# Spandan7724/Audio-Watermarking-Deep-Learning-Watermarks-for-Authenticating-Speech

Measured on AMD Instinct MI355X. Metric: 1-s@16kHz clips/sec (gen+det+loss fwd-bwd), higher is better.
Workload: dtype f32; 1 GPU; main16 train step: Generator+Detector+6 losses fwd-bwd + Adam, B=256 clips/GPU x 1 GPU, 1-s @ 16 kHz, message_bits=16 (BASELINE configs[2]); batch_per_gpu=256, global_batch=256, clip_len=16000, optimizer=fused flat Adam (wm_adam_step), parallelism=single

## Files before the change

### audio-watermarking-deep-learning-watermarks-for-authenticating-speech_amd/csrc/fft_lds.hpp

```cpp
#pragma once
#include "wm_common.hpp"

namespace wm {

__device__ __forceinline__ float2 cmul(float2 a, float2 b) { return make_float2(a.x * b.x - a.y * b.y, a.x * b.y + a.y * b.x); }

template <int LOGN>
__device__ __forceinline__ void fft_dif(float2* z, const float2* tw, int tid) {
    constexpr int N = 1 << LOGN;
#pragma unroll 1
    for (int st = 0; st < LOGN; ++st) {
        const int lm = LOGN - 1 - st, m = 1 << lm;
        for (int j = tid; j < N / 2; j += 256) {
            const int pos = j & (m - 1), i0 = ((j >> lm) << (lm + 1)) + pos, i1 = i0 + m;
            const float2 a = z[i0], b = z[i1], w = tw[pos << st];
            z[i0] = make_float2(a.x + b.x, a.y + b.y);
            z[i1] = cmul(make_float2(a.x - b.x, a.y - b.y), w);
        }
        __syncthreads();
    }
}
__device__ __forceinline__ double2 cmul(double2 a, double2 b) { return make_double2(a.x * b.x - a.y * b.y, a.x * b.y + a.y * b.x); }
template <int LOGN>
__device__ __forceinline__ void fft_dif(double2* z, const double2* tw, int tid) {
    constexpr int N = 1 << LOGN;
#pragma unroll 1
    for (int st = 0; st < LOGN; ++st) {
        const int lm = LOGN - 1 - st, m = 1 << lm;
        for (int j = tid; j < N / 2; j += 256) {
            const int pos = j & (m - 1), i0 = ((j >> lm) << (lm + 1)) + pos, i1 = i0 + m;
            const double2 a = z[i0], b = z[i1], w = tw[pos << st];
            z[i0] = make_double2(a.x + b.x, a.y + b.y);
            z[i1] = cmul(make_double2(a.x - b.x, a.y - b.y), w);
        }
        __syncthreads();
    }
}
template <int LOGN>
__device__ __forceinline__ int brev(int k) { return (int)(__brev((unsigned)k) >> (32 - LOGN)); }

}
```

### audio-watermarking-deep-learning-watermarks-for-authenticating-speech_amd/csrc/postproc.hip

```cpp
#include "wm_common.hpp"
using namespace wm;

namespace {

constexpr int kMaxTaps = 128;

__global__ __launch_bounds__(256) void postproc_fwd_kernel(const float* __restrict__ d_in, const float* __restrict__ taps,
                                                           int ntaps, float thr, float max_rms, float eps, int stages,
                                                           float* __restrict__ f_out, float* __restrict__ d_out,
                                                           float* __restrict__ stats, int T) {
    extern __shared__ __align__(16) float smem[];
    float* xs = smem;
    float* ks = smem + T + kMaxTaps;
    __shared__ float scratch[8];
    const int b = blockIdx.x, tid = threadIdx.x, pad = (ntaps - 1) / 2;
    const float* x = d_in + (size_t)b * T;
    const bool do_fir = stages & 1;
    for (int i = tid; i < T + 2 * pad; i += 256) {
        const int t = i - pad;
        xs[i] = (t >= 0 && t < T) ? x[t] : 0.f;
    }
    if (tid < ntaps) ks[tid] = taps[tid];
    __syncthreads();
    float ss = 0.f;
    for (int t = tid; t < T; t += 256) {
        float f;
        if (do_fir) {
            f = 0.f;
            for (int j = 0; j < ntaps; ++j) f = fmaf(ks[j], xs[t + j], f);
        } else {
            f = xs[t + pad];
        }
        if (f_out) f_out[(size_t)b * T + t] = f;
        const float cl = (stages & 2) ? fminf(fmaxf(f, -thr), thr) : f;
        d_out[(size_t)b * T + t] = cl;
        ss = fmaf(cl, cl, ss);
    }
    if (stages & 4) {
        const float tot = block_sum<4>(ss, scratch);
        const float cur = sqrtf(tot / (float)T + eps);
        const float gain = fminf(max_rms / cur, 1.0f);
        if (tid == 0 && stats) { stats[2 * b] = cur; stats[2 * b + 1] = gain; }
        for (int t = tid; t < T; t += 256) d_out[(size_t)b * T + t] *= gain;
    } else if (tid == 0 && stats) {
        stats[2 * b] = 0.f; stats[2 * b + 1] = 1.f;
    }
}

__global__ __launch_bounds__(256) void postproc_bwd_kernel(const float* __restrict__ g, const float* __restrict__ f_in,
                                                           const float* __restrict__ stats, const float* __restrict__ taps,
                                                           int ntaps, float thr, float max_rms, int stages,
                                                           float* __restrict__ d_raw, int T) {
    extern __shared__ __align__(16) float smem[];
    float* gs = smem;
    float* ks = smem + T + kMaxTaps;
    __shared__ float scratch[8];
    const int b = blockIdx.x, tid = threadIdx.x, pad = (ntaps - 1) / 2;
    const float* gb = g + (size_t)b * T;
    const float* fb = f_in + (size_t)b * T;
    if (tid < ntaps) ks[tid] = taps[tid];
    for (int i = tid; i < pad; i += 256) { gs[i] = 0.f; gs[pad + T + i] = 0.f; }
    float cur = 0.f, gain = 1.f;
    if (stages & 4) { cur = stats[2 * b]; gain = stats[2 * b + 1]; }
    float dot = 0.f;
    if ((stages & 4) && gain < 1.0f) {
        float acc = 0.f;
        for (int t = tid; t < T; t += 256) {
            const float f = fb[t];
            const float cl = (stages & 2) ? fminf(fmaxf(f, -thr), thr) : f;
            acc = fmaf(gb[t], cl, acc);
        }
        dot = block_sum<4>(acc, scratch);
    }
    const float r = max_rms / cur;
    const float kk = dot / ((float)T * cur * cur);
    for (int t = tid; t < T; t += 256) {
        const float f = fb[t];
        const float cl = (stages & 2) ? fminf(fmaxf(f, -thr), thr) : f;
        float dd = gb[t];
        if ((stages & 4) && gain < 1.0f) dd = r * (dd - cl * kk);
        if ((stages & 2) && !(f >= -thr && f <= thr)) dd = 0.f;
        gs[pad + t] = dd;
    }
    __syncthreads();
    for (int t = tid; t < T; t += 256) {
        float acc;
        if (stages & 1) {
            acc = 0.f;
            for (int j = 0; j < ntaps; ++j) acc = fmaf(ks[j], gs[t + 2 * pad - j], acc);
        } else {
            acc = gs[pad + t];
        }
        d_raw[(size_t)b * T + t] = acc;
    }
}

__global__ void embed_gather_kernel(const float* __restrict__ table, const long long* __restrict__ message,
                                    float* __restrict__ vec, int B, int nrows, int* __restrict__ err) {
    const int i = blockIdx.x * blockDim.x + threadIdx.x;
    if (i >= B * 64) return;
    const long long m = message[i >> 6];
    if (m < 0 || m >= nrows) { if (err) *err = 1; vec[i] = 0.f; return; }
    vec[i] = table[(size_t)m * 64 + (i & 63)];
}

__global__ __launch_bounds__(256) void embed_scatter_add_kernel(float* __restrict__ dtable, const long long* __restrict__ message,
                                                                const float* __restrict__ dvec, int B, int nrows) {
    const int lane = threadIdx.x & 63, b = blockIdx.x * 4 + (threadIdx.x >> 6);
    if (b >= B) return;
    const long long m = message[b];
    if (m < 0 || m >= nrows) return;
    float* row = dtable + (size_t)m * 64 + lane;
    float acc = 0.f;
    bool owner = false;
    for (int k0 = 0; k0 < B; k0 += 64) {
        const int idx = k0 + lane;
        const long long id = idx < B ? message[idx] : -1;
        unsigned long long hit = __ballot(id == m);
        if (k0 + 64 <= b) {
            if (hit) return;
            continue;
        }
        if (!owner) {
            const int sh = b - k0;
            if (hit & ((1ull << sh) - 1ull)) return;
            hit &= ~((1ull << sh) - 1ull);
            acc = *row;
            owner = true;
        }
        while (hit) {
            const int j = __builtin_ctzll(hit);
            hit &= hit - 1ull;
            acc += dvec[(size_t)(k0 + j) * 64 + lane];
        }
    }
    *row = acc;
}

__global__ __launch_bounds__(256) void rowsum_kernel(const float* __restrict__ x, float* __restrict__ out, int T4) {
    __shared__ float scratch[4];
    const float4* xr = reinterpret_cast<const float4*>(x) + (size_t)blockIdx.x * T4;
    float s = 0.f;
    for (int i = threadIdx.x; i < T4; i += 256) { const float4 v = xr[i]; s += (v.x + v.y) + (v.z + v.w); }
    s = block_sum<4>(s, scratch);
    if (threadIdx.x == 0) out[blockIdx.x] = s;
}

}

extern "C" {

int wm_postproc_fwd(const float* d_in, const float* taps, int ntaps, float thr, float max_rms, float eps, int stages,
                    float* f_out, float* d_out, float* stats, int B, int T, hipStream_t stream) {
    if (ntaps < 1 || ntaps > kMaxTaps || !(ntaps & 1) || T > 36000) return (int)hipErrorInvalidValue;
    const size_t lds = (size_t)(T + 2 * kMaxTaps) * sizeof(float);
    static size_t lds_set = 0;
    if (lds > lds_set) {
        WM_TRY(hipFuncSetAttribute(reinterpret_cast<const void*>(postproc_fwd_kernel), hipFuncAttributeMaxDynamicSharedMemorySize, (int)lds));
        lds_set = lds;
    }
    hipLaunchKernelGGL(postproc_fwd_kernel, dim3(B), dim3(256), lds, stream, d_in, taps, ntaps, thr, max_rms, eps, stages,
                       f_out, d_out, stats, T);
    WM_CHECK_LAUNCH();
    return 0;
}

int wm_postproc_bwd(const float* g, const float* f_in, const float* stats, const float* taps, int ntaps, float thr,
                    float max_rms, int stages, float* d_raw, int B, int T, hipStream_t stream) {
    if (ntaps < 1 || ntaps > kMaxTaps || !(ntaps & 1) || T > 36000) return (int)hipErrorInvalidValue;
    const size_t lds = (size_t)(T + 2 * kMaxTaps) * sizeof(float);
    static size_t lds_set = 0;
    if (lds > lds_set) {
        WM_TRY(hipFuncSetAttribute(reinterpret_cast<const void*>(postproc_bwd_kernel), hipFuncAttributeMaxDynamicSharedMemorySize, (int)lds));
        lds_set = lds;
    }
    hipLaunchKernelGGL(postproc_bwd_kernel, dim3(B), dim3(256), lds, stream, g, f_in, stats, taps, ntaps, thr, max_rms,
                       stages, d_raw, T);
    WM_CHECK_LAUNCH();
    return 0;
}

int wm_embed_gather(const float* table, const long long* message, float* vec, int B, int nrows, int* err, hipStream_t stream) {
    hipLaunchKernelGGL(embed_gather_kernel, dim3((B * 64 + 255) / 256), dim3(256), 0, stream, table, message, vec, B, nrows, err);
    WM_CHECK_LAUNCH();
    return 0;
}

int wm_embed_scatter_add(float* dtable, const long long* message, const float* dvec, int B, int nrows, hipStream_t stream) {
    if (B <= 0) return 0;
    hipLaunchKernelGGL(embed_scatter_add_kernel, dim3((B + 3) / 4), dim3(256), 0, stream, dtable, message, dvec, B, nrows);
    WM_CHECK_LAUNCH();
    return 0;
}

int wm_rowsum(const float* x, float* out, int rows, int T, hipStream_t stream) {
    if (T & 3) return (int)hipErrorInvalidValue;
    hipLaunchKernelGGL(rowsum_kernel, dim3(rows), dim3(256), 0, stream, x, out, T / 4);
    WM_CHECK_LAUNCH();
    return 0;
}

}
```

### audio-watermarking-deep-learning-watermarks-for-authenticating-speech_amd/csrc/stft_loss.hip

```cpp
#include "fft_lds.hpp"
using namespace wm;

namespace {

enum { MODE_MEL = 0, MODE_LOUD = 1, MODE_HF = 2 };

struct StftArgs {
    const float* a;
    const float* b;
    float* gframes;
    float* partial;
    const float* fb;
    const int* klo; const int* khi;
    const int* mlo;
    float gscale;
    float thresh;
    int kcut;
    int T, F, hop;
};

__device__ __forceinline__ int reflect_idx(int m, int T) {
    if (m < 0) m = -m;
    if (m >= T) m = 2 * (T - 1) - m;
    return m;
}

template <int LOGN, int MODE>
__global__ __launch_bounds__(256) void stft_loss_kernel(StftArgs p) {
    constexpr int N = 1 << LOGN, NB = N / 2 + 1;
    extern __shared__ __align__(16) float smem[];
    float2* z = reinterpret_cast<float2*>(smem);
    float2* tw = z + N;
    float2* GA = tw + N / 2;
    float2* GB = GA + NB;
    float* pw = reinterpret_cast<float*>(GB + NB);
    __shared__ float scratch[8];
    const int tid = threadIdx.x;
    const int units = (MODE == MODE_HF) ? (p.F + 1) / 2 : p.F;
    const int bclip = blockIdx.x / units, unit = blockIdx.x % units;
    const int fa = (MODE == MODE_HF) ? 2 * unit : unit;
    const int fbi = (MODE == MODE_HF) ? 2 * unit + 1 : unit;
    const bool b_valid = (MODE != MODE_HF) || (fbi < p.F);
    const float* sa = p.a + (size_t)bclip * p.T;
    const float* sb = (MODE == MODE_HF) ? sa : p.b + (size_t)bclip * p.T;

    for (int k = tid; k < N / 2; k += 256) {
        float s, c;
        sincospif(-2.0f * (float)k / (float)N, &s, &c);
        tw[k] = make_float2(c, s);
    }
    int differ = 0;
    for (int n = tid; n < N; n += 256) {
        const float w = 0.5f - 0.5f * cospif(2.0f * (float)n / (float)N);
        const float va = sa[reflect_idx(fa * p.hop + n - N / 2, p.T)];
        const float vb = b_valid ? sb[reflect_idx(fbi * p.hop + n - N / 2, p.T)] : 0.f;
        differ |= (va != vb);
        z[n] = make_float2(va * w, vb * w);
    }
    const bool same = (__syncthreads_or(differ) == 0) && MODE != MODE_HF;
    fft_dif<LOGN>(z, tw, tid);

    float loss = 0.f;
    for (int k = tid; k < NB; k += 256) {
        const float2 zk = z[brev<LOGN>(k)], zn = z[brev<LOGN>((N - k) & (N - 1))];
        const float2 A = make_float2(0.5f * (zk.x + zn.x), 0.5f * (zk.y - zn.y));
        const float2 Bv = make_float2(0.5f * (zk.y + zn.y), -0.5f * (zk.x - zn.x));
        if (MODE == MODE_MEL) {
            pw[k] = A.x * A.x + A.y * A.y;
            pw[NB + k] = Bv.x * Bv.x + Bv.y * Bv.y;
            GB[k] = Bv;
            GA[k] = make_float2(0.f, 0.f);
        } else if (MODE == MODE_LOUD) {
            const float ma = sqrtf(A.x * A.x + A.y * A.y), mb = sqrtf(Bv.x * Bv.x + Bv.y * Bv.y);
            const bool mask = ma > p.thresh;
            const float diff = same ? 0.f : mb - ma;
            if (mask) loss = fmaf(diff, diff, loss);
            const float coef = (mask && mb > 0.f) ? 2.0f * diff * p.gscale / mb : 0.f;
            GB[k] = make_float2(coef * Bv.x, coef * Bv.y);
            GA[k] = make_float2(0.f, 0.f);
        } else {
            float2 ga = make_float2(0.f, 0.f), gb = ga;
            if (k >= p.kcut) {
                const float ma = sqrtf(A.x * A.x + A.y * A.y), mb = sqrtf(Bv.x * Bv.x + Bv.y * Bv.y);
                loss += ma + mb;
                if (ma > 0.f) ga = make_float2(p.gscale * A.x / ma, p.gscale * A.y / ma);
                if (mb > 0.f) gb = make_float2(p.gscale * Bv.x / mb, p.gscale * Bv.y / mb);
            }
            GA[k] = ga;
            GB[k] = gb;
        }
    }
    if (MODE == MODE_MEL) {
        float* mel = pw + 2 * NB;
        float* dm = mel + 128;
        __syncthreads();
        if (tid < 128) {
            const int sig = tid >> 6, m = tid & 63;
            const float* pp = pw + sig * NB;
            float acc = 0.f;
            for (int k = p.klo[m]; k <= p.khi[m]; ++k) acc = fmaf(p.fb[k * 64 + m], pp[k], acc);
            mel[tid] = acc;
        }
        __syncthreads();
        if (tid < 64) {
            const float la = logf(mel[tid] + 1e-5f), lb = logf(mel[64 + tid] + 1e-5f);
            const float d = same ? 0.f : la - lb;
            loss = fabsf(d);
            const float sg = (d > 0.f) ? 1.f : ((d < 0.f) ? -1.f : 0.f);
            dm[tid] = -sg * p.gscale / (mel[64 + tid] + 1e-5f);
        }
        __syncthreads();
        for (int k = tid; k < NB; k += 256) {
            const int m0 = p.mlo[k];
            float dp = 0.f;
            for (int m = m0; m < m0 + 3 && m < 64; ++m) dp = fmaf(p.fb[k * 64 + m], dm[m], dp);
            const float2 Bv = GB[k];
            GB[k] = make_float2(2.0f * dp * Bv.x, 2.0f * dp * Bv.y);
        }
    }
    loss = block_sum<4>(loss, scratch);
    if (tid == 0) p.partial[blockIdx.x] = loss;
    if (!p.gframes) return;

    for (int k = tid; k < N; k += 256) {
        float2 ha, hb;
        if (k == 0 || k == N / 2) {
            ha = make_float2(GA[k].x, 0.f);
            hb = make_float2(GB[k].x, 0.f);
        } else if (k < N / 2) {
            ha = make_float2(0.5f * GA[k].x, 0.5f * GA[k].y);
            hb = make_float2(0.5f * GB[k].x, 0.5f * GB[k].y);
        } else {
            ha = make_float2(0.5f * GA[N - k].x, -0.5f * GA[N - k].y);
            hb = make_float2(0.5f * GB[N - k].x, -0.5f * GB[N - k].y);
        }
        z[k] = make_float2(ha.x - hb.y, -(ha.y + hb.x));
    }
    __syncthreads();
    fft_dif<LOGN>(z, tw, tid);
    float* ga_out = (MODE == MODE_HF) ? p.gframes + ((size_t)bclip * p.F + fa) * N : nullptr;
    float* gb_out = b_valid ? p.gframes + ((size_t)bclip * p.F + fbi) * N : nullptr;
    for (int n = tid; n < N; n += 256) {
        const float w = 0.5f - 0.5f * cospif(2.0f * (float)n / (float)N);
        const float2 y = z[brev<LOGN>(n)];
        if (ga_out) ga_out[n] = y.x * w;
        if (gb_out) gb_out[n] = -y.y * w;
    }
}

__global__ void ola_gather_kernel(const float* __restrict__ gframes, float* __restrict__ dsig, int N, int hop, int F,
                                  int T, int total, int accumulate) {
    const int i = blockIdx.x * blockDim.x + threadIdx.x;
    if (i >= total) return;
    const int b = i / T, t = i % T, half = N / 2;
    const float* gf = gframes + (size_t)b * F * N;
    int pos[3];
    int np = 0;
    pos[np++] = t + half;
    if (t >= 1 && t <= half) pos[np++] = half - t;
    if (t <= T - 2 && 2 * (T - 1) - t + half < T + N) { const int q = 2 * (T - 1) - t + half; if (q >= T + half) pos[np++] = q; }
    float acc = 0.f;
    for (int j = 0; j < np; ++j) {
        const int pp = pos[j];
        int f_hi = pp / hop;
        if (f_hi > F - 1) f_hi = F - 1;
        int f_lo = (pp - N + hop) / hop;
        if (pp - N + 1 <= 0) f_lo = 0;
        for (int f = f_lo; f <= f_hi; ++f) acc += gf[(size_t)f * N + (pp - f * hop)];
    }
    dsig[i] = accumulate ? dsig[i] + acc : acc;
}

template <int LOGN, int MODE>
int launch_stft(const StftArgs& p, int B, hipStream_t stream) {
    constexpr int N = 1 << LOGN, NB = N / 2 + 1;
    constexpr size_t lds = (size_t)(2 * N + N + 4 * NB + (MODE == MODE_MEL ? 2 * NB + 192 : 0)) * sizeof(float);
    const int units = (MODE == MODE_HF) ? (p.F + 1) / 2 : p.F;
    hipLaunchKernelGGL((stft_loss_kernel<LOGN, MODE>), dim3(B * units), dim3(256), lds, stream, p);
    WM_CHECK_LAUNCH();
    return 0;
}

}

extern "C" {

int wm_mel_loss(const float* clean, const float* wm, const float* fb, const int* klo, const int* khi, const int* mlo,
                float* gframes, float* partial, float* loss_out, float* dsig, int B, int T, hipStream_t stream) {
    const int N = 1024, hop = 256, F = 1 + T / hop;
    if (T <= N / 2) return (int)hipErrorInvalidValue;
    const double count = (double)B * 64.0 * F;
    StftArgs p{clean, wm, dsig ? gframes : nullptr, partial, fb, klo, khi, mlo, (float)(1.0 / count), 0.f, 0, T, F, hop};
    int rc = launch_stft<10, MODE_MEL>(p, B, stream);
    if (rc) return rc;
    rc = wm::launch_sum_scale2(partial, B * F, 1.0 / count, loss_out, stream);
    if (rc) return rc;
    if (dsig) {
        hipLaunchKernelGGL(ola_gather_kernel, dim3((B * T + 255) / 256), dim3(256), 0, stream, (const float*)gframes, dsig, N, hop, F, T, B * T, 0);
        WM_CHECK_LAUNCH();
    }
    return 0;
}

int wm_loud_loss(const float* clean, const float* wm, float thresh, float* gframes, float* partial, float* loss_out,
                 float* dsig, int B, int T, hipStream_t stream) {
    const int N = 2048, hop = 512, F = 1 + T / hop;
    if (T <= N / 2) return (int)hipErrorInvalidValue;
    const double count = (double)B * (N / 2 + 1) * F;
    StftArgs p{clean, wm, dsig ? gframes : nullptr, partial, nullptr, nullptr, nullptr, nullptr, (float)(1.0 / count), thresh, 0, T, F, hop};
    int rc = launch_stft<11, MODE_LOUD>(p, B, stream);
    if (rc) return rc;
    rc = wm::launch_sum_scale2(partial, B * F, 1.0 / count, loss_out, stream);
    if (rc) return rc;
    if (dsig) {
        hipLaunchKernelGGL(ola_gather_kernel, dim3((B * T + 255) / 256), dim3(256), 0, stream, (const float*)gframes, dsig, N, hop, F, T, B * T, 0);
        WM_CHECK_LAUNCH();
    }
    return 0;
}

int wm_hf_penalty(const float* delta, int kcut, float* gframes, float* partial, float* loss_out, float* dsig, int B, int T,
                  hipStream_t stream) {
    const int N = 512, hop = 128, F = 1 + T / hop;
    if (T <= N / 2) return (int)hipErrorInvalidValue;
    const double count = (double)B * (N / 2 + 1) * F;
    const int units = (F + 1) / 2;
    StftArgs p{delta, nullptr, dsig ? gframes : nullptr, partial, nullptr, nullptr, nullptr, nullptr, (float)(1.0 / count), 0.f, kcut, T, F, hop};
    int rc = launch_stft<9, MODE_HF>(p, B, stream);
    if (rc) return rc;
    rc = wm::launch_sum_scale2(partial, B * units, 1.0 / count, loss_out, stream);
    if (rc) return rc;
    if (dsig) {
        hipLaunchKernelGGL(ola_gather_kernel, dim3((B * T + 255) / 256), dim3(256), 0, stream, (const float*)gframes, dsig, N, hop, F, T, B * T, 0);
        WM_CHECK_LAUNCH();
    }
    return 0;
}

}
```

### include/wm_hip.h

```cpp
#ifndef WM_HIP_H
#define WM_HIP_H

#ifdef __cplusplus
extern "C" {
#endif

typedef struct ihipStream_t* wm_stream_t;


int wm_pack_w64(const float* w, float* wp, int KW, int mode, wm_stream_t stream);

int wm_conv64(const float* x, const float* x2, const float* wp, const float* pa, const float* pb, const float* pc,
              const float* bias, const float* e1, const float* ea, const float* eb, float* y, float* stats,
              int B, int T, int KW, int pro, int epi, wm_stream_t stream);

int wm_pack_w64_bf(const float* w, void* wpb, int mode, wm_stream_t stream);
int wm_set_conv_bf_schedule(int schedule, wm_stream_t stream);
int wm_conv64_bf(const float* x, const float* x2, const void* wpb, const float* pa, const float* pb, const float* pc,
                 const float* bias, const float* e1, const float* ea, const float* eb, float* y, float* stats,
                 int B, int T, int pro, int epi, int arith, wm_stream_t stream);
int wm_conv64_bf_tail(const float* x, const float* y2, const void* wpb_h, const float* sc2, const float* sh2, const float* bias,
                      float* out, void* mask, float* y, float* stats, int B, int T, wm_stream_t stream);

int wm_conv64_bf_stem(const float* s, const float* stem_w, const float* stem_b, const void* wpb_h, const float* bias, float* y0,
                      float* y, float* stats, int B, int T, wm_stream_t stream);

int wm_pack_w64_bf_scaled(const float* w, const float* row_scale, void* wpb, wm_stream_t stream);
int wm_resblock_eval_bf(const float* x, const void* w1pb, const void* w2pb, const float* b1, const float* sc1, const float* sh1,
                        const float* b2, const float* sc2, const float* sh2, float* y, int B, int T, int arith, wm_stream_t stream);
int wm_pack_w64_h_scaled(const float* w, const float* row_scale, void* wph, wm_stream_t stream);

int wm_dwgrad64_bf(const float* g, const float* g2, const float* ga, const float* gb, const float* gc, const void* wpb,
                   const float* x, const float* xa, const float* xb, const float* e1, const float* ea, const float* eb,
                   float* y, float* stats, float* partial, float* dw, float* dbias, int B, int T, int xpro, int epi, int accumulate,
                   const void* gmask, int arith, const float* gscale, float* dzmax, wm_stream_t stream);
int wm_pack_w64_h(const float* w, void* wph, int mode, wm_stream_t stream);
int wm_dwgrad64_bf_r1(const float* g, const float* g2, const float* ga, const float* gb, const float* gc, const void* wpb,
                      const float* x, const float* xa, const float* xb, const float* e1, const float* ea, const float* eb,
                      float* y, float* stats, float* partial, float* dw, float* dbias, int B, int T, int xpro, int epi, int accumulate,
                      const void* gmask, int arith, const float* gscale, float* dzmax, const float* g1, const float* hw,
                      wm_stream_t stream);
int wm_dwgrad64_bf_stem(const float* g, const float* g2, const float* ga, const float* gb, const float* gc, const void* wpb,
                        const float* e1, float* y, float* partial, float* dw, float* dbias, int B, int T, int accumulate,
                        const float* gscale, float* dzmax, const float* s, const float* stem_w, const float* stem_b,
                        wm_stream_t stream);

int wm_pack_w64_bf7(const float* w, void* wpb, int mode, wm_stream_t stream);
int wm_conv64_bf7(const float* x, const void* wpb, const float* vec, const float* bias, float* y, int B, int T, int pro, int epi,
                  int arith, const float* gscale, wm_stream_t stream);
int wm_pack_w64_h7(const float* w, void* wph, int mode, wm_stream_t stream);
int wm_gscale_absmax(const float* x, long long n, float* scratch, float log2_target, float* gscale, wm_stream_t stream);
int wm_gscale_from_max(const float* maxes, int n, float log2_target, float* gscale, wm_stream_t stream);
int wm_absmax_rows(const float* x, int rows, long long row_len, float* out, wm_stream_t stream);

int wm_wgrad64_bf7(const float* g, const float* x, const float* vec, float* partial, float* dw, float* dbias, int B, int T,
                   int xpro, int accumulate, int arith, const float* gscale, wm_stream_t stream);

int wm_wgrad64_bf(const float* g, const float* g2, const float* ga, const float* gb, const float* gc,
                  const float* x, const float* xa, const float* xb, float* partial, float* dw, float* dbias,
                  int B, int T, int gpro, int xpro, int accumulate, wm_stream_t stream);

int wm_wgrad64(const float* g, const float* g2, const float* ga, const float* gb, const float* gc,
               const float* x, const float* xa, const float* xb, float* partial, float* dw, float* dbias,
               int B, int T, int KW, int gpro, int xpro, int layout, int accumulate, wm_stream_t stream);

int wm_bn_finalize(const float* partials, int nparts, double count, const float* gamma, const float* beta,
                   float* running_mean, float* running_var, long long* num_batches_tracked, float momentum, float eps,
                   float* scale, float* shift, float* save_mean, float* save_invstd, wm_stream_t stream);
int wm_bn_eval_scale_shift(const float* gamma, const float* beta, const float* running_mean, const float* running_var,
                           float eps, float* scale, float* shift, wm_stream_t stream);
int wm_bn_add_relu(const float* x, const float* y2, const float* scale, const float* shift, float* out, int B, int T,
                   wm_stream_t stream);
int wm_relu_bwd_reduce(const float* g, const float* out, const float* y2, float* dz, float* partial, int B, int T,
                       wm_stream_t stream);
int wm_bn_add_relu_mask(const float* x, const float* y2, const float* scale, const float* shift, float* out, void* mask, int B, int T,
                        wm_stream_t stream);
int wm_relu_bwd_reduce_mask(const float* g, const void* mask, const float* y2, float* dz, float* partial, float* dzmax, int B, int T,
                            wm_stream_t stream);
int wm_relu_bwd_reduce_mask_r1(const float* g1, const float* w, const void* mask, const float* y2, float* partial, float* dzmax, int B,
                               int T, wm_stream_t stream);
int wm_bn_bwd_finalize(const float* partials, int nparts, double count, const float* gamma, const float* save_mean,
                       const float* save_invstd, float* A, float* Bc, float* Cc, float* dgamma, float* dbeta,
                       int accumulate, int eval_mode, const float* dzmax, int nmax, float* gscale, wm_stream_t stream);

int wm_stem_fwd(const float* s, const float* w, const float* bias, float* y, int B, int T, wm_stream_t stream);
int wm_stem_bwd(const float* g, const float* s, const float* w, float* ds, float* partial, float* dw, float* db, int B,
                int T, int nds, int accumulate, wm_stream_t stream);
int wm_head1_fwd(const float* x, const float* w, const float* bias, float* y, int B, int T, wm_stream_t stream);
int wm_head1_bwd(const float* g, const float* x, const float* w, float* dx, float* partial, float* dw, float* db, int B,
                 int T, int accumulate, wm_stream_t stream);
int wm_headN_fwd(const float* x, const float* w, const float* bias, float* y, int B, int T, int NO, wm_stream_t stream);
int wm_headN_bwd(const float* g, const float* x, const float* w, float* dx, float* partial, float* dw, float* db, int B,
                 int T, int NO, int accumulate, wm_stream_t stream);
int wm_head1_tail_fwd(const float* x, const float* y2, const float* scale, const float* shift, const float* w, const float* bias,
                      float* out, void* mask, float* y, int B, int T, wm_stream_t stream);
int wm_headN_tail_fwd(const float* x, const float* y2, const float* scale, const float* shift, const float* w, const float* bias,
                      const long long* message, int B, float* partial, float* loc_out, float* bce_out, float* out, void* mask,
                      float* logits, int R, int T, int NO, wm_stream_t stream);
int wm_headN_bwd_bce(const float* logits, const long long* message, const float* g_loc, const float* g_bce, const float* x,
                     const float* w, float* dx, float* partial, float* dw, float* db, int B, int R, int T, int NO, int accumulate,
                     wm_stream_t stream);

int wm_lstm_xproj(const float* x, const float* w_ih, const float* b_ih, const float* b_hh, float* xp, int B, int T,
                  wm_stream_t stream);
int wm_lstm_fwd(const float* xp, const float* w_hh, float* hout, float* gates, float* cst, int B, int T, wm_stream_t stream);
int wm_lstm_fwd_fused(const float* x, const float* w_ih, const float* b_ih, const float* b_hh, const float* w_hh,
                      float* hout, float* gates, float* cst, int B, int T, wm_stream_t stream);
int wm_set_lstm_fwd_wave_specialised(int on, wm_stream_t stream);
int wm_lstm_fwd_tail(const float* xres, const float* y2, const float* sc2, const float* sh2, float* out, void* mask, const float* w_ih,
                     const float* b_ih, const float* b_hh, const float* w_hh, float* hout, float* gates, float* cst, int B, int T,
                     wm_stream_t stream);
int wm_lstm_bwd(float* gates, const float* cst, const float* dh_out, const float* w_hh, int B, int T, wm_stream_t stream);
int wm_lstm_dx(const float* da, const float* w_ih, float* dx, int B, int T, wm_stream_t stream);
int wm_set_lstm_dx_bf16x6(int on, wm_stream_t stream);
int wm_lstm_bwd_fused(float* gates, const float* cst, const float* dh_out, const float* w_hh, const float* w_ih, float* dx,
                      int B, int T, wm_stream_t stream);
int wm_lstm_wgrad(const float* da, const float* x, const float* h, float* partial, float* dw_ih, float* dw_hh,
                  float* db_ih, float* db_hh, int B, int T, int accumulate, wm_stream_t stream);
int wm_lstm_bwd_wgrad(float* gates, const float* cst, const float* dh_out, const float* w_hh, const float* x, const float* h,
                      float* partial, float* dw_ih, float* dw_hh, float* db_ih, float* db_hh, int B, int T, int accumulate,
                      wm_stream_t stream);
int wm_lstm_bwd_wgrad_dx(const float* gates, const float* cst, const float* dh_out, const float* w_hh, const float* w_ih,
                         const float* x, const float* h, float* partial, float* dw_ih, float* dw_hh, float* db_ih, float* db_hh,
                         float* dx, int B, int T, int accumulate, wm_stream_t stream);

int wm_embed_gather(const float* table, const long long* message, float* vec, int B, int nrows, int* err, wm_stream_t stream);
int wm_embed_scatter_add(float* dtable, const long long* message, const float* dvec, int B, int nrows, wm_stream_t stream);
int wm_rowsum(const float* x, float* out, int rows, int T, wm_stream_t stream);

int wm_postproc_fwd(const float* d_in, const float* taps, int ntaps, float thr, float max_rms, float eps, int stages,
                    float* f_out, float* d_out, float* stats, int B, int T, wm_stream_t stream);
int wm_postproc_bwd(const float* g, const float* f_in, const float* stats, const float* taps, int ntaps, float thr,
                    float max_rms, int stages, float* d_raw, int B, int T, wm_stream_t stream);

int wm_mel_loss(const float* clean, const float* wm, const float* fb, const int* klo, const int* khi, const int* mlo,
                float* gframes, float* partial, float* loss_out, float* dsig, int B, int T, wm_stream_t stream);
int wm_loud_loss(const float* clean, const float* wm, float thresh, float* gframes, float* partial, float* loss_out,
                 float* dsig, int B, int T, wm_stream_t stream);
int wm_hf_penalty(const float* delta, int kcut, float* gframes, float* partial, float* loss_out, float* dsig, int B, int T,
                  wm_stream_t stream);

int wm_bce_fwd(const float* logits, const long long* message, float* partial, float* loc_out, float* bce_out, int B, int R,
               int T, int NO, wm_stream_t stream);
int wm_bce_bwd(const float* logits, const long long* message, const float* g_loc, const float* g_bce, float* dlogits, int B,
               int R, int T, int NO, wm_stream_t stream);
int wm_l1_fwd(const float* x, float* partial, float* out, long long n, wm_stream_t stream);
int wm_l1_bwd(const float* x, const float* g, float* dx, long long n, wm_stream_t stream);
int wm_adam_step(float* p, const float* g, float* m, float* v, long long n, double lr, double beta1, double beta2, double eps,
                 int step, wm_stream_t stream);

int wm_gconv(const float* x, const float* wp, const float* bias, const float* vec, const float* res, float* y, int NB,
             int Cin, int Lin, int K, int S, int P, int Mtot, int Nout, int st, int shp, int Cout, int Lout, int act,
             const float* x2, int Cin1, int nph, wm_stream_t stream);
int wm_gconv_h(const float* x, const void* wph, const float* bias, const float* vec, const float* res, float* y, int NB,
               int Cin, int Lin, int K, int S, int P, int Mtot, int Nout, int st, int shp, int Cout, int Lout, int act,
               const float* x2, int Cin1, int nph, const float* gscale, float* ymax, int per_clip, wm_stream_t stream);
int wm_gconv_pack_h(const float* wp, void* wph, float* scratch, int Cin, int K, int Mtot, wm_stream_t stream);
int wm_gconv_pack_h_conv(const float* w, void* wph, int Cout, int Cin, int K, int mode, wm_stream_t stream);
int wm_gwgrad_plan(int NB, int Ca, int Cb, int La, int K, long long* slab_floats, wm_stream_t stream);
int wm_gwgrad(const float* A, const float* Bx, float* G, float* dbias, float* slab, int NB, int Ca, int Cb, int La, int Lb,
              int K, int P, long long b_clip_stride, int remap, int r1, int r2, int accumulate, wm_stream_t stream);
int wm_gather_taps(const float* x, float* y, int NB, int C, int Lin, int K, int S, int P, int Lout, int order, wm_stream_t stream);
int wm_elu_bwd(const float* g, const float* y, float* dz, long long n, wm_stream_t stream);
int wm_channel_sum(const float* x, float* out, float* partial, int NB, int C, int L, int accumulate, wm_stream_t stream);
int wm_rowsum_any(const float* x, float* out, int rows, int L, wm_stream_t stream);
int wm_rows_scatter_add(float* dtable, const long long* idx, const float* dvec, int Bn, int dim, int nrows, wm_stream_t stream);
int wm_permute_acl(const float* x, float* y, int A, int C, int L, wm_stream_t stream);
int wm_lstm_seq_fwd(float* xp, const float* whh, float* hs, float* cs, int T, int H, int B, int save, wm_stream_t stream);
int wm_lstm_seq_bwd(float* gates, const float* cs, const float* dout, const float* whhT, float* dc, int T, int H, int B,
                    wm_stream_t stream);

int wm_resample_plan(int P, int Q, int width, int W, long long* tile_periods, wm_stream_t stream);
int wm_resample(const float* x, const float* taps, const int* first, float* y, int C, long long N, int P, int Q, int width, int W,
                long long L, long long total, wm_stream_t stream);

int wm_resample_add(const float* d, const float* taps, const int* first, const float* x, float* out, float* up, int C, long long N,
                    long long Nd, int P, int Q, int width, int W, wm_stream_t stream);

int wm_resample_rows(const float* x, const float* taps, const int* first, float* y, long long rows, long long N, long long L, int P, int Q,
                     int width, int W, wm_stream_t stream);

int wm_biquad_plan(int warm, int* chunk_len, wm_stream_t stream);
int wm_biquad(const float* x, void* out, void* mask_out, const void* mask_in, float b0, float b1, float b2, float a1, float a2,
              long long rows, long long n, int warm, int mode, int clamp, int reverse, wm_stream_t stream);

int wm_distort_plan(long long rows, long long n, long long* scratch_floats, wm_stream_t stream);
int wm_distort(const float* x, float* y, float* stat, float* scratch, long long rows, long long n, long long row0, long long seed,
               long long draw, float gain_lo, float gain_hi, float snr_lo, float snr_hi, float p_noise, wm_stream_t stream);
int wm_distort_bwd(const float* dy, const float* x, const float* stat, float* dx, float* scratch, long long rows, long long n,
                   long long row0, long long seed, long long draw, int through, wm_stream_t stream);

int wm_mdct_codec_plan(long long n, int M, int* frames_per_workgroup, long long* workgroups_per_row, wm_stream_t stream);
int wm_mdct_codec(const float* x, float* y, void* codes_out, const void* mask_in, const float* snr_db, long long rows, long long n, int M,
                  int band, int kcut, float floor_step, int quantise, wm_stream_t stream);

int wm_fir_rows(const float* x, const float* h, float* y, long long rows, long long n, int K, long long h_stride, int reverse,
                wm_stream_t stream);

int wm_rir_synth(const float* params, float* h, long long rows, int K, float sample_rate, long long row0, long long seed, long long draw,
                 wm_stream_t stream);

int wm_time_warp(const float* x, const float* params, const float* tab, float* y, long long rows, long long n, int zeros, int res,
                 int adjoint, wm_stream_t stream);

int wm_wsola(const float* x, const float* rate, const float* win, float* y, int* delta, long long rows, long long n_in, long long n_out,
             int L, int S, int mode, wm_stream_t stream);

int wm_lpc_codec(const float* x, float* y, const float* coeffs_in, float* coeffs_out, void* codes_out, const void* mask_in,
                 const float* snr_db, const float* lag, const float* expand, long long rows, long long n, int L, int p, float floor_step,
                 int quantise, int adjoint, wm_stream_t stream);

int wm_stoi_plan(long long rows, long long n, long long* scratch_bytes, wm_stream_t stream);
int wm_stoi(const float* x, const float* y, float* d, int* kept, void* scratch, long long rows, long long n, wm_stream_t stream);

int wm_masking_plan(long long rows, long long n, long long* frames, long long* chunk, long long* scratch_bytes, wm_stream_t stream);
int wm_masking_fwd(const float* x, const float* y, const float* tables, float* nmr_db, float* over_db, int* counts, float* coef,
                   void* scratch, long long rows, long long n, wm_stream_t stream);
int wm_masking_bwd(const float* x, const float* y, const float* coef, const float* gout, float* gy, long long rows, long long n,
                   wm_stream_t stream);

int wm_splice(const float* a, const float* b, float* y, int* lab, long long rows, long long n, long long row0, long long seed,
              long long draw, int max_spans, float p_span, long long len_lo, long long len_hi, float p_original, float p_silence,
              wm_stream_t stream);
int wm_splice_bwd(const float* dy, const int* lab, float* da, long long rows, long long n, wm_stream_t stream);
int wm_bce_masked_fwd(const float* logits, const long long* message, const int* lab, float* partial, long long* count_out,
                      float* loc_out, float* bce_out, int B, int R, int T, int NO, wm_stream_t stream);
int wm_bce_masked_bwd(const float* logits, const long long* message, const int* lab, const long long* count, const float* g_loc,
                      const float* g_bce, float* dlogits, int B, int R, int T, int NO, wm_stream_t stream);
int wm_loc_score(const float* logits, const int* lab, float thr_logit, int* counts, int* pred, int R, int T, int NO,
                 int lab_rows, wm_stream_t stream);

int wm_clip_scores_plan(long long R, int T, int NO, long long* scratch_bytes, wm_stream_t stream);
int wm_clip_scores(const float* logits, const long long* message, float thr_logit, float* prob, float* llr, int* votes, long long* words,
                   int* biterr, void* scratch, long long B, long long R, int T, int NO, wm_stream_t stream);

int wm_clip_features_plan(long long rows, long long n, int sample_rate, int* frames, int* energy_frames, int* lds_bytes,
                          wm_stream_t stream);
int wm_clip_features(const float* x, const float* sos, const float* fb, const int* klo, const int* khi, const float* dct, float* feat,
                     int* counts, float* frames_out, long long rows, long long n, int sample_rate, int warm, wm_stream_t stream);

int wm_noise_suppress_plan(long long rows, long long n, long long* frames, long long* scratch_bytes, wm_stream_t stream);
int wm_noise_suppress(const float* x, const float* src, const float* noise_in, const float* reduce_db, float* y,
                      float* gain_out, float* noise_out, void* scratch, long long rows, long long n,
                      float alpha, float over, wm_stream_t stream);

#ifdef __cplusplus
}
#endif
#endif
```

Measured before the change: 5820 clips/s.

## Add fast signal path: register-blocked FIR postproc, radix-4 FFT, cached twiddle tables

Adds 1024-thread postproc forward/backward kernels that compute the FIR four outputs per thread from vectorised LDS reads, with a version specialised for 101 taps. It also switches the STFT loss kernels to a radix-2² DIF FFT that halves the number of barrier-separated stages, and reads twiddles and the Hann window from precomputed device tables instead of calling sincos per block. The path is on by default and can be turned off with an env var or an API call. The risks are small floating-point differences from the changed FMA order, and a one-time host sync the first time the tables are built.

```diff
diff --git a/audio-watermarking-deep-learning-watermarks-for-authenticating-speech_amd/csrc/fft_lds.hpp b/audio-watermarking-deep-learning-watermarks-for-authenticating-speech_amd/csrc/fft_lds.hpp
--- a/audio-watermarking-deep-learning-watermarks-for-authenticating-speech_amd/csrc/fft_lds.hpp
+++ b/audio-watermarking-deep-learning-watermarks-for-authenticating-speech_amd/csrc/fft_lds.hpp
@@ -39,4 +39,38 @@
 template <int LOGN>
 __device__ __forceinline__ int brev(int k) { return (int)(__brev((unsigned)k) >> (32 - LOGN)); }
 
+__device__ __forceinline__ void bfly_dif(float2& a, float2& b, float2 w) {
+    const float2 d = make_float2(a.x - b.x, a.y - b.y);
+    a = make_float2(a.x + b.x, a.y + b.y);
+    b = make_float2(fmaf(d.x, w.x, -__fmul_rn(d.y, w.y)), fmaf(d.x, w.y, __fmul_rn(d.y, w.x)));
 }
+
+template <int LOGN, int ST = 0>
+__device__ __forceinline__ void fft_dif2(float2* z, const float2* tw, int tid) {
+    constexpr int N = 1 << LOGN;
+    if constexpr (ST + 1 < LOGN) {
+        constexpr int lm = LOGN - 1 - ST, m = 1 << lm, h = m >> 1;
+        for (int q = tid; q < N / 4; q += 256) {
+            const int pos = q & (h - 1), i0 = ((q >> (lm - 1)) << (lm + 1)) + pos;
+            float2 a = z[i0], b = z[i0 + h], c = z[i0 + m], d = z[i0 + m + h];
+            const float2 w2 = tw[pos << (ST + 1)];
+            bfly_dif(a, c, tw[pos << ST]);
+            bfly_dif(b, d, tw[(pos + h) << ST]);
+            bfly_dif(a, b, w2);
+            bfly_dif(c, d, w2);
+            z[i0] = a; z[i0 + h] = b; z[i0 + m] = c; z[i0 + m + h] = d;
+        }
+        __syncthreads();
+        fft_dif2<LOGN, ST + 2>(z, tw, tid);
+    } else if constexpr (ST < LOGN) {
+        const float2 w = tw[0];
+        for (int j = tid; j < N / 2; j += 256) {
+            float2 a = z[2 * j], b = z[2 * j + 1];
+            bfly_dif(a, b, w);
+            z[2 * j] = a; z[2 * j + 1] = b;
+        }
+        __syncthreads();
+    }
+}
+
+}
diff --git a/audio-watermarking-deep-learning-watermarks-for-authenticating-speech_amd/csrc/postproc.hip b/audio-watermarking-deep-learning-watermarks-for-authenticating-speech_amd/csrc/postproc.hip
--- a/audio-watermarking-deep-learning-watermarks-for-authenticating-speech_amd/csrc/postproc.hip
+++ b/audio-watermarking-deep-learning-watermarks-for-authenticating-speech_amd/csrc/postproc.hip
@@ -1,5 +1,7 @@
 #include "wm_common.hpp"
 using namespace wm;
+
+namespace wm { int signal_path_fast(); }
 
 namespace {
 
@@ -95,6 +97,178 @@
     }
 }
 
+constexpr int kFirThreads = 1024;
+constexpr size_t kFastLdsMax = (size_t)(36000 + 2 * kMaxTaps) * sizeof(float);
+
+__device__ __forceinline__ float first4_sum(float v, float* scratch) {
+    v = wave_sum(v);
+    const int lane = threadIdx.x & 63, w = threadIdx.x >> 6;
+    __syncthreads();
+    if (lane == 0 && w < 4) scratch[w] = v;
+    __syncthreads();
+    float r = 0.f;
+#pragma unroll
+    for (int i = 0; i < 4; ++i) r += scratch[i];
+    return r;
+}
+
+template <int NTAPS>
+__device__ __forceinline__ void fir4_fwd(const float* x, const float* ks, int nt, float (&f)[4]) {
+    if (NTAPS) nt = NTAPS;
+    const int groups = (nt + 3) >> 2;
+    f32x4 lo = lds_read4(x);
+    f[0] = f[1] = f[2] = f[3] = 0.f;
+#pragma unroll(NTAPS ? (NTAPS + 3) / 4 : 1)
+    for (int g = 0; g < groups; ++g) {
+        const f32x4 hi = lds_read4(x + 4 * (g + 1)), k4 = lds_read4(ks + 4 * g);
+        const float w[7] = {lo.x, lo.y, lo.z, lo.w, hi.x, hi.y, hi.z}, k[4] = {k4.x, k4.y, k4.z, k4.w};
+#pragma unroll
+        for (int u = 0; u < 4; ++u) {
+            if (4 * g + u < nt) {
+#pragma unroll
+                for (int r = 0; r < 4; ++r) f[r] = fmaf(k[u], w[r + u], f[r]);
+            }
+        }
+        lo = hi;
+    }
+}
+template <int NTAPS>
+__device__ __forceinline__ void fir4_bwd(const float* y, const float* ks, int nt, float (&f)[4]) {
+    if (NTAPS) nt = NTAPS;
+    const int groups = (nt + 3) >> 2;
+    const float* y0 = y - 4 * (groups - 1);
+    f32x4 hi = lds_read4(y0 + 4 * groups);
+    f[0] = f[1] = f[2] = f[3] = 0.f;
+#pragma unroll(NTAPS ? (NTAPS + 3) / 4 : 1)
+    for (int g = 0; g < groups; ++g) {
+        const f32x4 lo = lds_read4(y0 + 4 * (groups - 1 - g)), k4 = lds_read4(ks + 4 * g);
+        const float w[7] = {lo.x, lo.y, lo.z, lo.w, hi.x, hi.y, hi.z}, k[4] = {k4.x, k4.y, k4.z, k4.w};
+#pragma unroll
+        for (int u = 0; u < 4; ++u) {
+            if (4 * g + u < nt) {
+#pragma unroll
+                for (int r = 0; r < 4; ++r) f[r] = fmaf(k[u], w[3 + r - u], f[r]);
+            }
+        }
+        hi = lo;
+    }
+}
+
+template <int NTAPS>
+__global__ __launch_bounds__(kFirThreads) void postproc_fwd_fast_kernel(const float* __restrict__ d_in, const float* __restrict__ taps,
+                                                                        int ntaps, float thr, float max_rms, float eps, int stages,
+                                                                        float* __restrict__ f_out, float* __restrict__ d_out,
+                                                                        float* __restrict__ stats, int T) {
+    extern __shared__ __align__(16) float smem[];
+    float* xs = smem;
+    __shared__ __align__(16) float ks[kMaxTaps];
+    __shared__ float scratch[4];
+    const int b = blockIdx.x, tid = threadIdx.x, pad = (ntaps - 1) / 2;
+    const float* x = d_in + (size_t)b * T;
+    const bool do_fir = stages & 1;
+    for (int i = tid; i < T + 2 * pad; i += kFirThreads) {
+        const int t = i - pad;
+        xs[i] = (t >= 0 && t < T) ? x[t] : 0.f;
+    }
+    if (tid < ntaps) ks[tid] = taps[tid];
+    __syncthreads();
+    if (do_fir) {
+        const int nquads = (T + 3) >> 2;
+        for (int c0 = 0; c0 < nquads; c0 += kFirThreads) {
+            const int c = c0 + tid;
+            float f[4];
+            if (c < nquads) fir4_fwd<NTAPS>(xs + 4 * c, ks, ntaps, f);
+            __syncthreads();
+            if (c < nquads) reinterpret_cast<float4*>(xs)[c] = make_float4(f[0], f[1], f[2], f[3]);
+        }
+        __syncthreads();
+    }
+    const float* fs = do_fir ? xs : xs + pad;
+    float gain = 1.0f;
+    if (stages & 4) {
+        float ss = 0.f;
+        if (tid < 256) {
+            for (int t = tid; t < T; t += 256) {
+                const float f = fs[t];
+                const float cl = (stages & 2) ? fminf(fmaxf(f, -thr), thr) : f;
+                ss = fmaf(cl, cl, ss);
+            }
+        }
+        const float tot = first4_sum(ss, scratch);
+        const float cur = sqrtf(tot / (float)T + eps);
+        gain = fminf(max_rms / cur, 1.0f);
+        if (tid == 0 && stats) { stats[2 * b] = cur; stats[2 * b + 1] = gain; }
+    } else if (tid == 0 && stats) {
+        stats[2 * b] = 0.f; stats[2 * b + 1] = 1.f;
+    }
+    for (int t = tid; t < T; t += kFirThreads) {
+        const float f = fs[t];
+        if (f_out) f_out[(size_t)b * T + t] = f;
+        const float cl = (stages & 2) ? fminf(fmaxf(f, -thr), thr) : f;
+        d_out[(size_t)b * T + t] = (stages & 4) ? cl * gain : cl;
+    }
+}
+
+template <int NTAPS>
+__global__ __launch_bounds__(kFirThreads) void postproc_bwd_fast_kernel(const float* __restrict__ g, const float* __restrict__ f_in,
+                                                                        const float* __restrict__ stats, const float* __restrict__ taps,
+                                                                        int ntaps, float thr, float max_rms, int stages,
+                                                                        float* __restrict__ d_raw, int T) {
+    extern __shared__ __align__(16) float smem[];
+    __shared__ __align__(16) float ks[kMaxTaps];
+    __shared__ float scratch[4];
+    const int b = blockIdx.x, tid = threadIdx.x, pad = (ntaps - 1) / 2;
+    const int sh = (3 - 2 * pad) & 3;
+    float* gs = smem + sh;
+    const float* gb = g + (size_t)b * T;
+    const float* fb = f_in + (size_t)b * T;
+    if (tid < ntaps) ks[tid] = taps[tid];
+    for (int i = tid; i < pad; i += kFirThreads) { gs[i] = 0.f; gs[pad + T + i] = 0.f; }
+    float cur = 0.f, gain = 1.f;
+    if (stages & 4) { cur = stats[2 * b]; gain = stats[2 * b + 1]; }
+    float dot = 0.f;
+    if ((stages & 4) && gain < 1.0f) {
+        float acc = 0.f;
+        if (tid < 256) {
+            for (int t = tid; t < T; t += 256) {
+                const float f = fb[t];
+                const float cl = (stages & 2) ? fminf(fmaxf(f, -thr), thr) : f;
+                acc = fmaf(gb[t], cl, acc);
+            }
+        }
+        dot = first4_sum(acc, scratch);
+    }
+    const float r = max_rms / cur;
+    const float kk = dot / ((float)T * cur * cur);
+    for (int t = tid; t < T; t += kFirThreads) {
+        const float f = fb[t];
+        const float cl = (stages & 2) ? fminf(fmaxf(f, -thr), thr) : f;
+        float dd = gb[t];
+        if ((stages & 4) && gain < 1.0f) dd = r * (dd - cl * kk);
+        if ((stages & 2) && !(f >= -thr && f <= thr)) dd = 0.f;
+        gs[pad + t] = dd;
+    }
+    __syncthreads();
+    float* out = d_raw + (size_t)b * T;
+    if (stages & 1) {
+        const int nquads = (T + 3) >> 2, q0 = (2 * pad + sh - 3) >> 2;
+        const bool vec = (reinterpret_cast<uintptr_t>(out) & 15) == 0;
+        for (int c = tid; c < nquads; c += kFirThreads) {
+            float f[4];
+            fir4_bwd<NTAPS>(smem + 4 * (c + q0), ks, ntaps, f);
+            if (vec && 4 * c + 3 < T) {
+                *reinterpret_cast<float4*>(out + 4 * c) = make_float4(f[0], f[1], f[2], f[3]);
+            } else {
+#pragma unroll
+                for (int k = 0; k < 4; ++k)
+                    if (4 * c + k < T) out[4 * c + k] = f[k];
+            }
+        }
+    } else {
+        for (int t = tid; t < T; t += kFirThreads) out[t] = gs[pad + t];
+    }
+}
+
 __global__ void embed_gather_kernel(const float* __restrict__ table, const long long* __restrict__ message,
                                     float* __restrict__ vec, int B, int nrows, int* __restrict__ err) {
     const int i = blockIdx.x * blockDim.x + threadIdx.x;
@@ -154,6 +328,15 @@
                     float* f_out, float* d_out, float* stats, int B, int T, hipStream_t stream) {
     if (ntaps < 1 || ntaps > kMaxTaps || !(ntaps & 1) || T > 36000) return (int)hipErrorInvalidValue;
     const size_t lds = (size_t)(T + 2 * kMaxTaps) * sizeof(float);
+    if (wm::signal_path_fast()) {
+        static wm::DevOnce done[2];
+        if (int rc = wm::lds_opt_in(reinterpret_cast<const void*>(postproc_fwd_fast_kernel<101>), kFastLdsMax, done[0])) return rc;
+        if (int rc = wm::lds_opt_in(reinterpret_cast<const void*>(postproc_fwd_fast_kernel<0>), kFastLdsMax, done[1])) return rc;
+        if (ntaps == 101) hipLaunchKernelGGL(postproc_fwd_fast_kernel<101>, dim3(B), dim3(kFirThreads), lds, stream, d_in, taps, ntaps, thr, max_rms, eps, stages, f_out, d_out, stats, T);
+        else hipLaunchKernelGGL(postproc_fwd_fast_kernel<0>, dim3(B), dim3(kFirThreads), lds, stream, d_in, taps, ntaps, thr, max_rms, eps, stages, f_out, d_out, stats, T);
+        WM_CHECK_LAUNCH();
+        return 0;
+    }
     static size_t lds_set = 0;
     if (lds > lds_set) {
         WM_TRY(hipFuncSetAttribute(reinterpret_cast<const void*>(postproc_fwd_kernel), hipFuncAttributeMaxDynamicSharedMemorySize, (int)lds));
@@ -169,6 +352,15 @@
                     float max_rms, int stages, float* d_raw, int B, int T, hipStream_t stream) {
     if (ntaps < 1 || ntaps > kMaxTaps || !(ntaps & 1) || T > 36000) return (int)hipErrorInvalidValue;
     const size_t lds = (size_t)(T + 2 * kMaxTaps) * sizeof(float);
+    if (wm::signal_path_fast()) {
+        static wm::DevOnce done[2];
+        if (int rc = wm::lds_opt_in(reinterpret_cast<const void*>(postproc_bwd_fast_kernel<101>), kFastLdsMax, done[0])) return rc;
+        if (int rc = wm::lds_opt_in(reinterpret_cast<const void*>(postproc_bwd_fast_kernel<0>), kFastLdsMax, done[1])) return rc;
+        if (ntaps == 101) hipLaunchKernelGGL(postproc_bwd_fast_kernel<101>, dim3(B), dim3(kFirThreads), lds, stream, g, f_in, stats, taps, ntaps, thr, max_rms, stages, d_raw, T);
+        else hipLaunchKernelGGL(postproc_bwd_fast_kernel<0>, dim3(B), dim3(kFirThreads), lds, stream, g, f_in, stats, taps, ntaps, thr, max_rms, stages, d_raw, T);
+        WM_CHECK_LAUNCH();
+        return 0;
+    }
     static size_t lds_set = 0;
     if (lds > lds_set) {
         WM_TRY(hipFuncSetAttribute(reinterpret_cast<const void*>(postproc_bwd_kernel), hipFuncAttributeMaxDynamicSharedMemorySize, (int)lds));
diff --git a/audio-watermarking-deep-learning-watermarks-for-authenticating-speech_amd/csrc/stft_loss.hip b/audio-watermarking-deep-learning-watermarks-for-authenticating-speech_amd/csrc/stft_loss.hip
--- a/audio-watermarking-deep-learning-watermarks-for-authenticating-speech_amd/csrc/stft_loss.hip
+++ b/audio-watermarking-deep-learning-watermarks-for-authenticating-speech_amd/csrc/stft_loss.hip
@@ -1,5 +1,8 @@
 #include "fft_lds.hpp"
+#include <stdlib.h>
 using namespace wm;
+
+namespace wm { int signal_path_fast(); }
 
 namespace {
 
@@ -19,13 +22,38 @@
     int T, F, hop;
 };
 
+struct SignalTables {
+    static constexpr int kTw = 256 + 512 + 1024, kWin = 512 + 1024 + 2048;
+    __host__ __device__ static constexpr int tw_off(int logn) { return (1 << (logn - 1)) - 256; }
+    __host__ __device__ static constexpr int win_off(int logn) { return (1 << logn) - 512; }
+};
+__device__ float2 g_signal_tw[SignalTables::kTw];
+__device__ float g_signal_win[SignalTables::kWin];
+
+__global__ __launch_bounds__(256) void signal_tables_kernel(int logn, float2* tw, float* win) {
+    const int N = 1 << logn, n = blockIdx.x * 256 + threadIdx.x;
+    if (!tw) tw = g_signal_tw + SignalTables::tw_off(logn);
+    if (!win) win = g_signal_win + SignalTables::win_off(logn);
+    if (n < N / 2) {
+        float s, c;
+        sincospif(-2.0f * (float)n / (float)N, &s, &c);
+        tw[n] = make_float2(c, s);
+    }
+    if (n < N) win[n] = 0.5f - 0.5f * cospif(2.0f * (float)n / (float)N);
+}
+__global__ __launch_bounds__(256) void signal_tables_read_kernel(int logn, float2* tw, float* win) {
+    const int N = 1 << logn, n = blockIdx.x * 256 + threadIdx.x;
+    if (n < N / 2) tw[n] = g_signal_tw[SignalTables::tw_off(logn) + n];
+    if (n < N) win[n] = g_signal_win[SignalTables::win_off(logn) + n];
+}
+
 __device__ __forceinline__ int reflect_idx(int m, int T) {
     if (m < 0) m = -m;
     if (m >= T) m = 2 * (T - 1) - m;
     return m;
 }
 
-template <int LOGN, int MODE>
+template <int LOGN, int MODE, bool FAST>
 __global__ __launch_bounds__(256) void stft_loss_kernel(StftArgs p) {
     constexpr int N = 1 << LOGN, NB = N / 2 + 1;
     extern __shared__ __align__(16) float smem[];
@@ -44,21 +72,27 @@
     const float* sa = p.a + (size_t)bclip * p.T;
     const float* sb = (MODE == MODE_HF) ? sa : p.b + (size_t)bclip * p.T;
 
+    const float* win = g_signal_win + SignalTables::win_off(LOGN);
     for (int k = tid; k < N / 2; k += 256) {
-        float s, c;
-        sincospif(-2.0f * (float)k / (float)N, &s, &c);
-        tw[k] = make_float2(c, s);
+        if constexpr (FAST) {
+            tw[k] = g_signal_tw[SignalTables::tw_off(LOGN) + k];
+        } else {
+            float s, c;
+            sincospif(-2.0f * (float)k / (float)N, &s, &c);
+            tw[k] = make_float2(c, s);
+        }
     }
     int differ = 0;
     for (int n = tid; n < N; n += 256) {
-        const float w = 0.5f - 0.5f * cospif(2.0f * (float)n / (float)N);
+        const float w = FAST ? win[n] : 0.5f - 0.5f * cospif(2.0f * (float)n / (float)N);
         const float va = sa[reflect_idx(fa * p.hop + n - N / 2, p.T)];
         const float vb = b_valid ? sb[reflect_idx(fbi * p.hop + n - N / 2, p.T)] : 0.f;
         differ |= (va != vb);
         z[n] = make_float2(va * w, vb * w);
     }
     const bool same = (__syncthreads_or(differ) == 0) && MODE != MODE_HF;
-    fft_dif<LOGN>(z, tw, tid);
+    if constexpr (FAST) fft_dif2<LOGN>(z, tw, tid);
+    else fft_dif<LOGN>(z, tw, tid);
 
     float loss = 0.f;
     for (int k = tid; k < NB; k += 256) {
@@ -137,11 +171,12 @@
         z[k] = make_float2(ha.x - hb.y, -(ha.y + hb.x));
     }
     __syncthreads();
-    fft_dif<LOGN>(z, tw, tid);
+    if constexpr (FAST) fft_dif2<LOGN>(z, tw, tid);
+    else fft_dif<LOGN>(z, tw, tid);
     float* ga_out = (MODE == MODE_HF) ? p.gframes + ((size_t)bclip * p.F + fa) * N : nullptr;
     float* gb_out = b_valid ? p.gframes + ((size_t)bclip * p.F + fbi) * N : nullptr;
     for (int n = tid; n < N; n += 256) {
-        const float w = 0.5f - 0.5f * cospif(2.0f * (float)n / (float)N);
+        const float w = FAST ? win[n] : 0.5f - 0.5f * cospif(2.0f * (float)n / (float)N);
         const float2 y = z[brev<LOGN>(n)];
         if (ga_out) ga_out[n] = y.x * w;
         if (gb_out) gb_out[n] = -y.y * w;
@@ -171,19 +206,62 @@
     dsig[i] = accumulate ? dsig[i] + acc : acc;
 }
 
+wm::DevOnce g_tables_built;
+int ensure_signal_tables(hipStream_t stream) {
+    if (wm::dev_done(g_tables_built)) return 0;
+    for (int logn = 9; logn <= 11; ++logn) {
+        hipLaunchKernelGGL(signal_tables_kernel, dim3((1 << logn) / 256), dim3(256), 0, stream, logn, (float2*)nullptr, (float*)nullptr);
+        WM_CHECK_LAUNCH();
+    }
+    WM_TRY(hipStreamSynchronize(stream));
+    wm::dev_mark(g_tables_built);
+    return 0;
+}
+
 template <int LOGN, int MODE>
 int launch_stft(const StftArgs& p, int B, hipStream_t stream) {
     constexpr int N = 1 << LOGN, NB = N / 2 + 1;
     constexpr size_t lds = (size_t)(2 * N + N + 4 * NB + (MODE == MODE_MEL ? 2 * NB + 192 : 0)) * sizeof(float);
     const int units = (MODE == MODE_HF) ? (p.F + 1) / 2 : p.F;
-    hipLaunchKernelGGL((stft_loss_kernel<LOGN, MODE>), dim3(B * units), dim3(256), lds, stream, p);
+    if (MODE != MODE_HF && wm::signal_path_fast()) {
+        if (int rc = ensure_signal_tables(stream)) return rc;
+        hipLaunchKernelGGL((stft_loss_kernel<LOGN, MODE, MODE != MODE_HF>), dim3(B * units), dim3(256), lds, stream, p);
+    } else {
+        hipLaunchKernelGGL((stft_loss_kernel<LOGN, MODE, false>), dim3(B * units), dim3(256), lds, stream, p);
+    }
     WM_CHECK_LAUNCH();
     return 0;
 }
 
 }
 
+static std::atomic<int> g_signal_path{-1};
+int wm::signal_path_fast() {
+    int v = g_signal_path.load(std::memory_order_relaxed);
+    if (v < 0) {
+        const char* e = getenv("WM_SIGNAL_PATH");
+        v = (e && e[0] == '0' && e[1] == '\0') ? 0 : 1;
+        g_signal_path.store(v, std::memory_order_relaxed);
+    }
+    return v;
+}
+
 extern "C" {
+
+int wm_set_signal_path(int fast, hipStream_t) { g_signal_path.store(fast ? 1 : 0, std::memory_order_relaxed); return 0; }
+
+int wm_signal_tables(int n_fft, int from_tables, float* tw, float* win, hipStream_t stream) {
+    const int logn = n_fft == 512 ? 9 : n_fft == 1024 ? 10 : n_fft == 2048 ? 11 : 0;
+    if (!logn || !tw || !win) return (int)hipErrorInvalidValue;
+    if (from_tables) {
+        if (int rc = ensure_signal_tables(stream)) return rc;
+        hipLaunchKernelGGL(signal_tables_read_kernel, dim3(n_fft / 256), dim3(256), 0, stream, logn, reinterpret_cast<float2*>(tw), win);
+    } else {
+        hipLaunchKernelGGL(signal_tables_kernel, dim3(n_fft / 256), dim3(256), 0, stream, logn, reinterpret_cast<float2*>(tw), win);
+    }
+    WM_CHECK_LAUNCH();
+    return 0;
+}
 
 int wm_mel_loss(const float* clean, const float* wm, const float* fb, const int* klo, const int* khi, const int* mlo,
                 float* gframes, float* partial, float* loss_out, float* dsig, int B, int T, hipStream_t stream) {
diff --git a/include/wm_hip.h b/include/wm_hip.h
--- a/include/wm_hip.h
+++ b/include/wm_hip.h
@@ -139,6 +139,8 @@
                  float* dsig, int B, int T, wm_stream_t stream);
 int wm_hf_penalty(const float* delta, int kcut, float* gframes, float* partial, float* loss_out, float* dsig, int B, int T,
                   wm_stream_t stream);
+int wm_set_signal_path(int fast, wm_stream_t stream);
+int wm_signal_tables(int n_fft, int from_tables, float* tw, float* win, wm_stream_t stream);
 
 int wm_bce_fwd(const float* logits, const long long* message, float* partial, float* loc_out, float* bce_out, int B, int R,
                int T, int NO, wm_stream_t stream);
```

Result: no change. 5860 clips/s (median of 6 runs) (+0.7%).
